# Icelk/fractal-renderer

Measured on AMD Instinct MI355X. Metric: pixel_iterations_per_sec, higher is better.
Workload: dtype f64

## Files before the change

### fractal-renderer_amd/csrc/fr_api.hip

```cpp
#include <hip/hip_runtime.h>

#include <atomic>
#include <cmath>
#include <cstddef>
#include <cstdint>
#include <cstdio>
#include <cstdlib>
#include <cstring>
#include <mutex>
#include <shared_mutex>
#include <string>
#include <vector>

#include "fr_ctx.h"

static_assert(sizeof(fr_config) == 104 && offsetof(fr_config, limit) == 16 && offsetof(fr_config, inside) == 72 &&
                  offsetof(fr_config, primary_color) == 74 && offsetof(fr_config, color_weight) == 80 &&
                  offsetof(fr_config, julia_set) == 88,
              "fr_config must stay the #[repr(C)] image of calc::Config");
static_assert(sizeof(fr_render_opts) == 32, "fr_render_opts is part of the ABI");

namespace fr {

namespace {
// ... 358 lines not shown
            slot_cv.notify_all();
        }
        s->busy = true;
        pending = s->pending;
        s->pending = false;
    }
    if (pending) e = hipEventSynchronize(s->done);
    if (e != hipSuccess) {
        {
            std::lock_guard<std::mutex> lk(palette_mu);
            s->busy = false;
        }
        slot_cv.notify_all();
        return fail_hip(e, "survivor-list buffer");
    }
    *out = s;
    return FR_OK;
}

void Ctx::release_surv(SurvSlot *slot, hipStream_t st) {
    if (!slot) return;
    const bool recorded = slot->done && hipEventRecord(slot->done, st) == hipSuccess;
    if (!recorded) (void)hipStreamSynchronize(st);
    {
        std::lock_guard<std::mutex> lk(palette_mu);
        slot->pending = recorded;
        slot->busy = false;
    }
    slot_cv.notify_all();
}

namespace {

int init_primary_locked(int device) {
    int n = 0;
    hipError_t e = hipGetDeviceCount(&n);
    if (e != hipSuccess || n <= 0) {
        (void)hipGetLastError();
        return fail(FR_ERR_NO_DEVICE, "no HIP device available (libfractal_hip has no CPU fallback)");
    }
    if (device < 0) device = g_primary_inited ? g_primary.hip_device : 0;
    if (device >= n) return fail(FR_ERR_NO_DEVICE, "device index out of range");
    if (g_primary_inited && g_primary.hip_device == device) return FR_OK;
    if (g_primary_inited) {
        g_primary.destroy();
        g_primary_inited = false;
    }
    static std::once_flag once;
    std::call_once(once, [] { atexit([] { g_process_exiting.store(true); }); });
    int rc = g_primary.create(device);
    if (rc != FR_OK) {
        g_primary.destroy();
        return rc;
    }
    g_primary_inited = true;
    return FR_OK;
}

}

int primary(Ctx **out) {
    {
        std::lock_guard<std::mutex> lk(g_primary_mu);
        if (!g_primary_inited) {
            int rc = init_primary_locked(-1);
            if (rc != FR_OK) return rc;
        }
    }
    HIP_TRY(hipSetDevice(g_primary.hip_device));
    *out = &g_primary;
    return FR_OK;
}

Ctx *primary_if_created() {
    std::lock_guard<std::mutex> lk(g_primary_mu);
    return g_primary_inited ? &g_primary : nullptr;
}

void fill_params(const fr_config *cfg, const Opts &o, fr_kparams &p) {
    memset(&p, 0, sizeof p);
    p.algo = cfg->algo;
    p.width = cfg->width;
    p.height = cfg->height;
    p.iterations = cfg->iterations;
    p.limit = cfg->limit;
    p.stable_limit = cfg->stable_limit;
    p.pos_re = cfg->pos.re;
    p.pos_im = cfg->pos.im;
    p.scale_re = cfg->scale.re;
    p.scale_im = cfg->scale.im;
    p.exposure = cfg->exposure;
    p.julia_re = cfg->julia_set.re;
    p.julia_im = cfg->julia_set.im;
    p.inside = cfg->inside ? 1u : 0u;
    p.smooth = cfg->smooth ? 1u : 0u;
    p.prim[0] = cfg->primary_color.r;
    p.prim[1] = cfg->primary_color.g;
    p.prim[2] = cfg->primary_color.b;
    p.sec[0] = cfg->secondary_color.r;
    p.sec[1] = cfg->secondary_color.g;
    p.sec[2] = cfg->secondary_color.b;
    for (int k = 0; k < 3; k++) {
        p.prim_f[k] = (double)p.prim[k];
        p.sec_f[k] = (double)p.sec[k];
    }
    p.iterations_f64 = (double)cfg->iterations;
    const uint32_t n = cfg->iterations;
    p.inv_iterations = (n != 0 && (n & (n - 1)) == 0) ? 1.0 / (double)n : 0.0;
    p.ncols = cfg->width;
    p.nrows = 0;
    p.x_first = 0;
    p.x_stride = 1;
    p.block_rows = 1;
    p.y_first = 0;
    p.y_stride = 1;
    p.refill_minrun = o.refill_minrun < 0 ? 32u : (uint32_t)o.refill_minrun;
    p.refill_quit16 = o.refill_quit16 < 0 ? 8u : (uint32_t)o.refill_quit16;
    p.queue_minrun = (o.refill_minrun < 0 || (o.tile >= 11 && o.tile <= 16)) ? 8u : (uint32_t)o.refill_minrun;
    p.first_keep = ((o.tile >= 11 && o.tile <= 16) && o.refill_quit16 > 0) ? 4u * (uint32_t)o.refill_quit16 : 0u;
    p.two_pass_cap = ((o.tile >= 11 && o.tile <= 16) && o.refill_minrun > 0) ? (uint32_t)o.refill_minrun : 0u;
    p.queue_want = (o.refill_quit16 < 0 || (o.tile >= 11 && o.tile <= 16)) ? 24u : (64u * (uint32_t)o.refill_quit16 + 15u) / 16u;
    {
        static const int dbg_want = getenv("FR_DEBUG_QUEUE_WANT") ? atoi(getenv("FR_DEBUG_QUEUE_WANT")) : 0;
        static const int dbg_minrun = getenv("FR_DEBUG_QUEUE_MINRUN") ? atoi(getenv("FR_DEBUG_QUEUE_MINRUN")) : -1;
        if (dbg_want > 0 && dbg_want <= 64) p.queue_want = (uint32_t)dbg_want;
        if (dbg_minrun >= 0) p.queue_minrun = (uint32_t)dbg_minrun;
    }
    {
        static const int dbg_ablate = getenv("FR_DEBUG_ABLATE") ? atoi(getenv("FR_DEBUG_ABLATE")) : 0;
        p.debug_ablate = (uint32_t)dbg_ablate & 3u;
    }
    p.cycle_shortcut = (o.cycle_shortcut && cfg->iterations < (1u << 30)) ? 1u : 0u;
    p.filt_k = n != 0 ? cfg->exposure / (double)n : 0.0;
    const bool filter_ok = o.colour_filter && cfg->smooth && n != 0 && std::isfinite(cfg->exposure) &&
                           std::fabs(p.filt_k) <= 1e100 && cfg->stable_limit >= 0.0;
    p.colour_filter = filter_ok ? 1u : 0u;
    const double ak = std::fabs(p.filt_k);
    p.colour_filter32 = (filter_ok && o.colour_filter == 1 && n < (1u << 24) && ak >= 0x1p-60 && ak <= 0x1p60) ? 1u : 0u;
    p.filt_k32 = (float)p.filt_k;
    p.filt_c32 = p.colour_filter32 ? std::nextafterf((float)(ak * FR_NU_BRACKET * (1.0 + 0x1p-9)), INFINITY) : 0.0f;
    for (int k = 0; k < 3; k++) {
        p.filt_d[k] = p.prim_f[k] * ak * FR_NU_BRACKET * (1.0 + 0x1p-20);
        p.filt_d32[k] = p.colour_filter32 ? std::nextafterf((float)(p.prim_f[k] * ak * FR_NU_BRACKET * (1.0 + 0x1p-10)), INFINITY) : 0.0f;
        p.prim32[k] = (float)p.prim[k];
    }
    const double lo = std::fmax(cfg->stable_limit, 2.0) * (1.0 + 0x1p-20);
    p.filt_lo32 = (p.colour_filter32 && lo < 1e30) ? std::nextafterf((float)lo, INFINITY) : INFINITY;
}

void rows_params(const fr_config *cfg, const Opts &o, uint32_t y0, uint32_t y1, unsigned channels, fr_kparams &p) {
    fill_params(cfg, o, p);
    p.nrows = y1 - y0;
    p.y_first = y0;
    p.block_rows = p.nrows;
    p.y_stride = 0;
    p.out_rgba = channels == 4 ? 1u : 0u;
}

static double host_coord(double coord, double max, double offset, double pos, double scale) {
    return ((coord / max) - offset) / scale + pos;
}

constexpr uint32_t kSpecQuiet = 16;
constexpr uint32_t kSpecBlock = 16, kSpecMaxLen = 128;

static uint32_t spec_maxlen() {
// ... 1220 lines not shown
```

### fractal-renderer_amd/csrc/fr_kernels.h

```cpp
#ifndef FR_KERNELS_H
#define FR_KERNELS_H

#include <hip/hip_runtime.h>
#include <stdint.h>

struct fr_kparams {
    uint32_t algo;
    uint32_t width, height;
    uint32_t iterations;
    double limit, stable_limit;
    double pos_re, pos_im, scale_re, scale_im;
    double exposure;
    double julia_re, julia_im;
    uint32_t inside, smooth;
    uint32_t prim[3], sec[3];
    double prim_f[3], sec_f[3];
    double iterations_f64, inv_iterations;
    uint32_t ncols, nrows;
    uint32_t x_first, x_stride;
    uint32_t block_rows, y_first, y_stride;
    uint32_t out_in_place;
    uint32_t out_rgba;
    uint32_t loop_mode;
    double skip_t;
    uint32_t loop_spec;
    uint32_t loop_spec_max;
    uint32_t first_no_spec;
    const uint32_t *palette;
    uint32_t palette_entries;
    uint32_t refill_minrun, refill_quit16;
    uint32_t queue_minrun, queue_want;
    uint32_t cycle_shortcut;
    uint32_t colour_filter;
    uint32_t *work_counter;
    double filt_k;
    double filt_d[3];
    uint32_t colour_filter32;
    float filt_k32;
    float filt_c32;
    float filt_d32[3];
    float prim32[3];
    float filt_lo32;
    uint32_t first_cap;
    uint32_t first_keep;
    uint32_t two_pass_cap;
    uint32_t first_only;
    uint32_t second_v1;
    uint32_t first_one_band;
    uint32_t strip_tiles;
    uint32_t debug_ablate;
    uint32_t surv_sub_capacity;
    void *surv_z;
    uint32_t *surv_pos;
    uint32_t *surv_cnt;
    void *surv_c;
    uint32_t *surv_counts;
};

constexpr uint32_t FR_SURV_QUEUES = 64;
constexpr uint32_t FR_SURV_COUNT_STRIDE = 32;
constexpr uint32_t FR_SURV_CHUNK = 64;

constexpr double FR_NU_BRACKET = 0x1p-18;

enum fr_out_mode {
    FR_OUT_RGB = 0,
    FR_OUT_ESCAPE = 1,
    FR_OUT_COUNT = 2
};

constexpr uint32_t FR_COUNT_SLOTS = 512;

constexpr int kDeepWaves = 4;
constexpr int kDeepTileW = 8, kDeepTileH = 8;
constexpr int kDeepWavesX = 2, kDeepWavesY = 2;
constexpr int kDeepBlockW = kDeepTileW * kDeepWavesX, kDeepBlockH = kDeepTileH * kDeepWavesY;

struct fr_kout {
    uint8_t *rgb;
    double *z;
    uint32_t *iters;
    unsigned long long *count;
    unsigned long long *trace;
};

inline hipError_t fr_deep_grid(const fr_kparams &p, dim3 &grid, dim3 &block) {
    const uint64_t tiles = (((uint64_t)p.ncols + kDeepBlockW - 1) / kDeepBlockW) * (((uint64_t)p.nrows + kDeepBlockH - 1) / kDeepBlockH);
    if (tiles > 0x7FFFFFFFull) return hipErrorInvalidValue;
    grid = dim3((uint32_t)tiles);
    block = dim3(64 * kDeepWaves);
    return hipSuccess;
}

hipError_t fr_launch_escape(const fr_kparams &p, int precision, int mode, const fr_kout &out, int tile,
                            hipStream_t stream, const char **kernel_name);

hipError_t fr_launch_escape_dd(const fr_kparams &p, double pos_lo_re, double pos_lo_im, int mode, const fr_kout &out,
                               bool with_lo, hipStream_t stream, const char **kernel_name);

bool fr_wants_work_queue(const fr_kparams &p, int tile);

bool fr_wants_two_pass(fr_kparams &p, int precision, int tile, int hint = -1);
struct fr_two_pass_layout {
    size_t z_off, pos_off, cnt_off, c_off, counts_off, total;
};
fr_two_pass_layout fr_two_pass_bytes(const fr_kparams &p, int precision, uint32_t sub_capacity);

hipError_t fr_launch_view_sample(const fr_kparams &p, int precision, uint32_t side, uint32_t cap_s, uint32_t episode, uint32_t keep,
                                 unsigned long long *counters, unsigned long long *result, unsigned long long tag,
                                 hipStream_t stream);

hipError_t fr_launch_copy_out(const void *src, void *dst, size_t bytes, unsigned int *counter, unsigned long long *flag,
                              unsigned long long seq, hipStream_t stream);

constexpr uint32_t FR_MAX_PALETTE_ENTRIES = 1280;

hipError_t fr_launch_palette(const fr_kparams &p, uint32_t *palette, hipStream_t stream);

hipError_t fr_launch_colour(const fr_kparams &p, const double *z, const uint32_t *iters, size_t n, uint8_t *rgb,
                            hipStream_t stream);

hipError_t fr_launch_escape_extend(const fr_kparams &p, int precision, uint32_t from_iterations, double *z, uint32_t *iters,
                                   hipStream_t stream, const char **kernel_name);
hipError_t fr_launch_escape_extend_dd(const fr_kparams &p, double pos_lo_re, double pos_lo_im, uint32_t from_iterations,
                                      double *z, uint32_t *iters, hipStream_t stream, const char **kernel_name);

hipError_t fr_launch_colour_rows(const fr_kparams &p, const double *z, uint32_t z_width, const uint32_t *iters, size_t n,
                                 uint32_t channels, void *out, hipStream_t stream);

hipError_t fr_launch_box_filter(const void *src, uint32_t width, uint64_t rows, uint32_t s, uint32_t bpp, void *dst,
                                hipStream_t stream);

hipError_t fr_launch_colour_filter(const fr_kparams &p, const double *z, uint32_t z_width, const uint32_t *iters, uint32_t width,
                                   uint64_t rows, uint32_t s, uint32_t bpp, void *dst, hipStream_t stream);

hipError_t fr_launch_view_stats(const double *z, uint32_t z_width, const uint32_t *iters, size_t n, double stable_limit,
                                uint32_t iterations, void *stats, hipStream_t stream);

hipError_t fr_launch_recursive_batch(uint32_t iterations, const double *start, const double *c, size_t n,
// ... 11 lines not shown
```

### fractal-renderer_amd/csrc/fr_kernels.hip

```cpp
#include "fr_kernels.h"

#include <cmath>

#include <cstdlib>

#include "fr_launch.h"
#include "fr_math.h"

namespace {

#include "fr_colour.h"

constexpr int kWaves = 4;



#define FR_ORBIT_IT_R(SFX, S, D)                           \
    "v_add_" SFX " %[t], %[r2" S "], -%[i2" S "]\n"        \
    "v_add_" SFX " %[x], %[re" S "], %[re" S "]\n"         \
    "v_add_" SFX " %[re" D "], %[t], %[cre]\n"             \
    "v_mul_" SFX " %[x], %[x], %[im" S "]\n"               \
    "v_add_" SFX " %[im" D "], %[x], %[cim]\n"             \
    "v_mul_" SFX " %[r2" D "], %[re" D "], %[re" D "]\n"   \
    "v_mul_" SFX " %[i2" D "], %[im" D "], %[im" D "]\n"
// ... 319 lines not shown
    "v_cmp_lt_" SFX " vcc, %[t4lim], %[t]\n"                                       \
    "s_cbranch_vccnz .Lslow_%=\n"                                                  \
    SP_ARM                                                                         \
    "s_branch .Lfast_%=\n"                                                         \
    FR_ORBIT_RECORD("R", "0") SLOW_RECORDS CYC_H SP_BODY                           \
    ".Ldone_%=:\n"                                                                 \
    "s_mov_b64 exec, %[sorig]\n"

#define FR_SC_CYC_CHECK(EQ, TAG)                   \
    EQ " %[scyc], %[X], %[Xs]\n"                   \
    EQ " vcc, %[Y], %[Ys]\n"                       \
    "s_and_b64 %[scyc], %[scyc], vcc\n"            \
    "s_cbranch_scc1 .Lcyc" TAG "_%=\n"             \
    ".Lcyccont" TAG "_%=:\n"                       \
    "s_cmp_ge_u32 %[si], %[snext]\n"               \
    "s_cbranch_scc1 .Lsave" TAG "_%=\n"            \
    ".Lsavecont" TAG "_%=:\n"

#define FR_SC_CYC_SAVE(MOV, TAG)                   \
    ".Lsave" TAG "_%=:\n"                          \
    MOV " %[Xs], %[X]\n"                           \
    MOV " %[Ys], %[Y]\n"                           \
    "v_mov_b32 %[vsaved], %[si]\n"                 \
    "s_lshl_b32 %[snext], %[snext], 1\n"           \
    "s_branch .Lsavecont" TAG "_%=\n"

#define FR_SC_CYC_HANDLER(TAG)                     \
    ".Lcyc" TAG "_%=:\n"                           \
    "s_or_b32 %[stmp], %[si], 0x80000000\n"        \
    "s_mov_b64 %[sprev], exec\n"                   \
    "s_mov_b64 exec, %[scyc]\n"                    \
    "v_mov_b32 %[it], %[stmp]\n"                   \
    "s_andn2_b64 exec, %[sprev], %[scyc]\n"        \
    "s_cbranch_execz .Ldone_%=\n"                  \
    "s_bcnt1_i32_b64 %[scnt], exec\n"              \
    "s_cmp_gt_u32 %[scnt], %[thr]\n"               \
    "s_cbranch_scc1 .Lcyccont" TAG "_%=\n"         \
    "s_cmp_lt_u32 %[si], %[minrun]\n"              \
    "s_cbranch_scc1 .Lcyccont" TAG "_%=\n"         \
    "s_branch .Ldone_%=\n"

#define FR_SC_ASM_M4_(SFX, CYC_F, CYC_S, CYC_H, SP_INIT, SP_ARM, SP_ENTRY, SP_BODY)                 \
    FR_SC_ASM(SFX, "4", FR_SC_ITS4(SFX),                    \
              FR_SC_CHECKED_STEP(SFX, "A") FR_SC_CHECKED_STEP(SFX, "B") FR_SC_CHECKED_STEP(SFX, "C") \
                  FR_SC_CHECKED_STEP(SFX, "D"),                                                     \
              FR_ORBIT_RECORD("A", "0") FR_ORBIT_RECORD("B", "1") FR_ORBIT_RECORD("C", "2")         \
                  FR_ORBIT_RECORD("D", "3"),                                                        \
              CYC_F, CYC_S, CYC_H, SP_INIT, SP_ARM, SP_ENTRY, SP_BODY)
#define FR_SC_ASM_M2_(SFX, CYC_F, CYC_S, CYC_H)                                            \
    FR_SC_ASM(SFX, "2", FR_SC_ITS2(SFX),                                        \
              FR_SC_CHECKED_STEP(SFX, "A") FR_SC_CHECKED_STEP(SFX, "B"),                    \
              FR_ORBIT_RECORD("A", "0") FR_ORBIT_RECORD("B", "1"), CYC_F, CYC_S, CYC_H, "", "", FR_SC_NOSPEC_ENTRY, "")
#define FR_SC_ASM_M4(SFX) FR_SC_ASM_M4_(SFX, "", "", "", "", "", FR_SC_NOSPEC_ENTRY, "")
#define FR_SC_ASM_M2(SFX) FR_SC_ASM_M2_(SFX, "", "", "")
#define FR_SC_ASM_M4_SPEC(SFX, MOV)                                                                 \
    FR_SC_ASM_M4_(SFX, "", "", "", "s_min_u32 %[sspec], %[specq], %[n]\n" "s_max_u32 %[lcap], %[lcap], " FR_SPEC_MSTR "\n", FR_SC_SPEC_ARM, FR_SC_SPEC_ENTRY(FR_SPEC_MSTR), \
                  FR_SC_SPEC_BODY(SFX, MOV, FR_SPEC_MSTR, FR_SC_SPEC_REST))
#define FR_SC_CYC_HANDLERS(MOV) \
    FR_SC_CYC_HANDLER("F") FR_SC_CYC_HANDLER("S") FR_SC_CYC_SAVE(MOV, "F") FR_SC_CYC_SAVE(MOV, "S")
#define FR_SC_ASM_M4_CYC(SFX, EQ, MOV) \
    FR_SC_ASM_M4_(SFX, FR_SC_CYC_CHECK(EQ, "F"), FR_SC_CYC_CHECK(EQ, "S"), FR_SC_CYC_HANDLERS(MOV), "", "", FR_SC_NOSPEC_ENTRY, "")
#define FR_SC_ASM_M2_CYC(SFX, EQ, MOV) \
    FR_SC_ASM_M2_(SFX, FR_SC_CYC_CHECK(EQ, "F"), FR_SC_CYC_CHECK(EQ, "S"), FR_SC_CYC_HANDLERS(MOV))

template <typename T>
struct ScalableRange;
template <>
struct ScalableRange<double> {
    static constexpr double lo = 0x1p-300, hi = 0x1p400;
};
template <>
struct ScalableRange<float> {
    static constexpr float lo = 0x1p-30f, hi = 0x1p30f;
};

template <typename T>
__device__ __forceinline__ bool lane_is_scalable(T re0, T im0, T cre, T cim) {
    constexpr T lo = ScalableRange<T>::lo, hi = ScalableRange<T>::hi;
    auto c_ok = [=](T v) { return __builtin_fabs(v) >= lo && __builtin_fabs(v) <= hi; };
    auto s_ok = [=](T v) { return v == (T)0 || c_ok(v); };
    return c_ok(cre) && c_ok(cim) && s_ok(re0) && s_ok(im0);
}

template <typename T, int M, bool CYC>
__device__ __forceinline__ uint32_t orbit_scaled_run(uint32_t iterations, T &X, T &Y, T &A, T &B, T c2re, T c2im,
                                                     T squared, T skip_t, EpisodeCtl ctl, uint32_t &completed,
                                                     T *pXs = nullptr, T *pYs = nullptr,
                                                     uint32_t *saved_index = nullptr, uint32_t spec_quiet = 0u,
                                                     uint32_t spec_maxlen = 0u) {
    uint32_t it;
    T t, q;
    T X1, Y1, A1, B1;
    uint32_t sspec;
    uint32_t specq = __builtin_amdgcn_readfirstlane(spec_quiet ? spec_quiet : 0xFFFFFFFFu);
    uint32_t lcap = __builtin_amdgcn_readfirstlane(spec_maxlen);
    T Xs = CYC ? *pXs : T(0), Ys = CYC ? *pYs : T(0);
    uint32_t vsaved = 0xFFFFFFFFu;
    uint32_t snext = 32u;
    unsigned long long sorig, sprev, sdiff, scyc;
    uint32_t si, stmp, nrem, scnt;
    const uint32_t n = __builtin_amdgcn_readfirstlane(iterations);
    const uint32_t thr = __builtin_amdgcn_readfirstlane(ctl.thr), minrun = __builtin_amdgcn_readfirstlane(ctl.minrun);
    const T lim4_v = (T)4 * squared, t4_v = (T)4 * skip_t;
#define FR_SC_OUTPUTS                                                                                           \
    [X] "+v"(X), [Y] "+v"(Y), [A] "+v"(A), [B] "+v"(B), [it] "=&v"(it), [t] "=&v"(t), [q] "=&v"(q),             \
        [sorig] "=&s"(sorig), [sprev] "=&s"(sprev), [sdiff] "=&s"(sdiff), [si] "=&s"(si), [stmp] "=&s"(stmp),   \
        [nrem] "=&s"(nrem), [scnt] "=&s"(scnt)
#define FR_SC_INPUTS                                                                                            \
    [c2re] "v"(c2re), [c2im] "v"(c2im), [lim4] "s"(lim4), [t4lim] "s"(t4lim), [n] "s"(n), [thr] "s"(thr),       \
        [minrun] "s"(minrun)
#define FR_SC_OPERANDS : FR_SC_OUTPUTS : FR_SC_INPUTS : "vcc", "scc"
#define FR_SC_OPERANDS_SPEC                                                                                     \
    : FR_SC_OUTPUTS, [X1] "=&v"(X1), [Y1] "=&v"(Y1), [A1] "=&v"(A1), [B1] "=&v"(B1), [sspec] "=&s"(sspec),      \
      [specq] "+&s"(specq), [lcap] "+&s"(lcap)                                                                  \
    : FR_SC_INPUTS                                                                                              \
    : "vcc", "scc"
#define FR_SC_OPERANDS_CYC                                                                                      \
    : FR_SC_OUTPUTS, [scyc] "=&s"(scyc), [Xs] "+v"(Xs), [Ys] "+v"(Ys), [vsaved] "+v"(vsaved), [snext] "+s"(snext) \
    : FR_SC_INPUTS                                                                                              \
    : "vcc", "scc"
    const auto lim4 = uniform_bits<T>(lim4_v), t4lim = uniform_bits<T>(t4_v);
    if constexpr (sizeof(T) == 8) {
        if constexpr (M == 4 && CYC)
            asm volatile(FR_SC_ASM_M4_CYC("f64", "v_cmp_eq_u64", "v_mov_b64") FR_SC_OPERANDS_CYC);
        else if constexpr (M == 4)
            asm volatile(FR_SC_ASM_M4_SPEC("f64", "v_mov_b64") FR_SC_OPERANDS_SPEC);
        else if constexpr (CYC)
            asm volatile(FR_SC_ASM_M2_CYC("f64", "v_cmp_eq_u64", "v_mov_b64") FR_SC_OPERANDS_CYC);
        else
            asm volatile(FR_SC_ASM_M2("f64") FR_SC_OPERANDS);
    } else {
        if constexpr (M == 4 && CYC)
            asm volatile(FR_SC_ASM_M4_CYC("f32", "v_cmp_eq_u32", "v_mov_b32") FR_SC_OPERANDS_CYC);
        else if constexpr (M == 4)
            asm volatile(FR_SC_ASM_M4_SPEC("f32", "v_mov_b32") FR_SC_OPERANDS_SPEC);
        else if constexpr (CYC)
            asm volatile(FR_SC_ASM_M2_CYC("f32", "v_cmp_eq_u32", "v_mov_b32") FR_SC_OPERANDS_CYC);
        else
            asm volatile(FR_SC_ASM_M2("f32") FR_SC_OPERANDS);
    }
    (void)scyc;
    (void)snext;
    (void)X1, (void)Y1, (void)A1, (void)B1, (void)sspec, (void)specq, (void)lcap;
    if constexpr (CYC) {
        *pXs = Xs;
        *pYs = Ys;
        *saved_index = vsaved;
    }
    completed = si;
    return it;
}

template <typename T, int M>
__device__ __forceinline__ uint32_t orbit_scaled(uint32_t iterations, T &re, T &im, T cre, T cim, T squared,
                                                 T skip_t, T &r2, T &i2, uint32_t spec_quiet = 0u, uint32_t spec_maxlen = 0u) {
    T X = re + re, Y = im + im, A = X * X, B = Y * Y;
    uint32_t completed;
    const uint32_t it = orbit_scaled_run<T, M, false>(iterations, X, Y, A, B, cre + cre, cim + cim, squared, skip_t,
                                               EpisodeCtl{0, 0}, completed, nullptr, nullptr, nullptr, spec_quiet, spec_maxlen);
    re = X * (T)0.5;
    im = Y * (T)0.5;
    r2 = re * re;
    i2 = im * im;
    return it;
}

template <typename T>
__device__ __forceinline__ uint32_t orbit_auto(uint32_t loop_mode, uint32_t iterations, T &re, T &im, T cre, T cim,
                                               T squared, T skip_t, T &r2, T &i2, int strip_scalable = -1,
                                               uint32_t spec_quiet = 0u, uint32_t spec_maxlen = 0u) {
    if (loop_mode != 0 && strip_scalable != 0) {
        bool all_ok = strip_scalable == 1;
        if (strip_scalable < 0) all_ok = __ballot(!lane_is_scalable<T>(re, im, cre, cim)) == 0ull;
        if (all_ok) {
            if (loop_mode == 4) return orbit_scaled<T, 4>(iterations, re, im, cre, cim, squared, skip_t, r2, i2, spec_quiet, spec_maxlen);
            return orbit_scaled<T, 2>(iterations, re, im, cre, cim, squared, skip_t, r2, i2);
        }
    }
    return orbit<T>(iterations, re, im, cre, cim, squared, r2, i2, spec_quiet);
}

__device__ __forceinline__ double coord_to_space(double coord, double max, double offset, double pos,
                                                 double scale) {
    return ((coord / max) - offset) / scale + pos;
}

__device__ __forceinline__ void store_pixel(uint32_t ncols, uint32_t out_rgba, uint8_t *base, uint32_t row, uint32_t col,
                                            const uint8_t rgb[3]) {
    const uint64_t k = (uint64_t)row * ncols + col;
    if (out_rgba) {
        reinterpret_cast<uint32_t *>(base)[k] =
            (uint32_t)rgb[0] | ((uint32_t)rgb[1] << 8) | ((uint32_t)rgb[2] << 16) | 0xFF000000u;
    } else {
        uint8_t *o = base + 3ull * k;
        o[0] = rgb[0];
        o[1] = rgb[1];
        o[2] = rgb[2];
    }
}
__device__ __forceinline__ void store_pixel(const fr_kparams &p, uint8_t *base, uint32_t row, uint32_t col, const uint8_t rgb[3]) {
    store_pixel(p.ncols, p.out_rgba, base, row, col, rgb);
}

typedef const __attribute__((address_space(4))) fr_kparams *KArgs;
#define FR_COLD_PARAMS(NAME)                                                          \
    KArgs NAME = (KArgs)__builtin_amdgcn_kernarg_segment_ptr();  \
    asm volatile("" : "+s"(NAME))

__device__ __forceinline__ unsigned long long ballot64(bool b) { return __builtin_amdgcn_ballot_w64(b); }

__device__ __forceinline__ bool lane_in(unsigned long long m) { return __builtin_amdgcn_inverse_ballot_w64(m); }

struct Filter32 {
    float lo, k, c, p0, p1, p2;
};
__device__ __forceinline__ uint32_t cvt_pk_u8_at(float v, uint32_t acc, int K) {
    return __builtin_amdgcn_cvt_pk_u8_f32(v, (uint32_t)K, acc);
}
__device__ __forceinline__ bool colour_fast32(const Filter32 &f, float d32, float itp1, uint32_t &lo) {
    const float l1 = __builtin_amdgcn_logf(d32);
    const float nu32 = __builtin_amdgcn_logf(l1 * 0.25f);
    const float m = (itp1 - nu32) * f.k;
    const float w = __builtin_fmaf(__builtin_fabsf(m), 0x1p-20f, f.c);
    const float ml = m - w, mh = m + w;
    lo = cvt_pk_u8_at(__builtin_fmaf(f.p2, ml, -0.5f), cvt_pk_u8_at(__builtin_fmaf(f.p1, ml, -0.5f), cvt_pk_u8_at(__builtin_fmaf(f.p0, ml, -0.5f), 0u, 0), 1), 2);
    const uint32_t hi = cvt_pk_u8_at(__builtin_fmaf(f.p2, mh, -0.5f), cvt_pk_u8_at(__builtin_fmaf(f.p1, mh, -0.5f), cvt_pk_u8_at(__builtin_fmaf(f.p0, mh, -0.5f), 0u, 0), 1), 2);
    return lo == hi;
}

__device__ __forceinline__ void store_packed(uint8_t *base, uint32_t off, uint32_t packed, uint32_t bpp) {
    if (bpp == 4u) {
        const uint32_t v = packed | 0xFF000000u;
        asm volatile("s_nop 4\n\tglobal_store_dword %0, %1, %2" : : "v"(off), "v"(v), "s"(base) : "memory");
    } else {
        asm volatile("s_nop 4\n\tglobal_store_short %0, %1, %2\n\tglobal_store_byte_d16_hi %0, %1, %2 offset:2" : : "v"(off), "v"(packed), "s"(base) : "memory");
    }
}

struct TileOut {
    uint8_t *base;
    uint32_t lane_off, bpp;
    bool narrow, fast_colour;
};

template <typename T>
__device__ __forceinline__ uint32_t colour_packed(bool valid, bool fast_colour, T re, T im, T r2, T i2, uint32_t iters,
                                                  const double *lds_tab, const uint32_t *palette) {
    uint32_t packed = 0;
    unsigned long long todo = ballot64(valid);
    if (fast_colour) {
        Filter32 f;
        {
            FR_COLD_PARAMS(kp);
            f.lo = kp->filt_lo32, f.k = kp->filt_k32, f.c = kp->filt_c32;
            f.p0 = kp->prim32[0], f.p1 = kp->prim32[2], f.p2 = kp->prim32[1];
        }
        float d32;
        if constexpr (sizeof(T) == 8)
            d32 = (float)(r2 + i2);
        else
            d32 = r2 + i2;
        const unsigned long long outside = ballot64(valid && d32 >= f.lo);
        if (outside != 0ull) {
            uint32_t pk;
            const bool decided = colour_fast32(f, d32, (float)(iters + 1u), pk);
            const bool ok = lane_in(outside) && d32 <= 0x1.ffffep119f && decided;
            packed = ok ? pk : 0u;
            todo &= ~ballot64(ok);
        }
    }
    if (todo != 0ull) {
        bool inside_done = false;
        if (lane_in(todo)) {
            double dist;
            if constexpr (sizeof(T) == 8) {
                dist = (double)(r2 + i2);
            } else {
                const double zre = (double)re, zim = (double)im;
                dist = zre * zre + zim * zim;
            }
            FR_COLD_PARAMS(kp);
            inside_done = !(dist > kp->stable_limit);
            if (inside_done && kp->inside)
                packed = sat_u8_dev(kp->sec_f[0] * dist) | (sat_u8_dev(kp->sec_f[2] * dist) << 8) | (sat_u8_dev(kp->sec_f[1] * dist) << 16);
        }
        todo &= ~ballot64(inside_done);
    }
    if (todo != 0ull) {
        if (lane_in(todo)) {
            FR_COLD_PARAMS(kp);
            const ColourConsts cc = make_colour_consts(*kp);
            uint8_t rgb[3];
            colour_pixel<T>(cc, re, im, r2, i2, iters, lds_tab, palette, rgb);
            packed = (uint32_t)rgb[0] | ((uint32_t)rgb[1] << 8) | ((uint32_t)rgb[2] << 16);
        }
    }
    return packed;
}

template <typename T, int MODE>
__device__ __forceinline__ void render_pixel(const fr_kparams &p, const fr_kout &out, const double *s_tab,
                                             const uint32_t *s_pal, double sre, double sim, bool valid,
                                             uint32_t cx, uint32_t r, uint32_t lane, uint32_t r_out,
                                             int strip_scalable = -1, const TileOut *to = nullptr) {
    double zre = 0.0, zim = 0.0;
    T tre = 0, tim = 0, tr2 = 0, ti2 = 0;
    uint32_t iters = 0;
    const bool escape_algo = p.algo == 0  || p.algo == 2 ;
    if (valid && escape_algo) {
        const double cre = p.algo == 0 ? sre : p.julia_re;
        const double cim = p.algo == 0 ? sim : p.julia_im;
        if constexpr (sizeof(T) == 8) {
            tre = sre;
            tim = sim;
            iters = orbit_auto<double>(p.loop_mode, p.iterations, tre, tim, cre, cim, p.limit * p.limit, p.skip_t,
                                       tr2, ti2, strip_scalable, p.loop_spec, p.loop_spec_max);
            zre = tre;
            zim = tim;
        } else {
            tre = (float)sre, tim = (float)sim;
            const float lim = (float)p.limit;
            iters = orbit_auto<float>(p.loop_mode, p.iterations, tre, tim, (float)cre, (float)cim, lim * lim,
                                      (float)p.skip_t, tr2, ti2, strip_scalable, p.loop_spec, p.loop_spec_max);
            zre = (double)tre;
            zim = (double)tim;
        }
    }

    if constexpr (MODE == FR_OUT_RGB) {
        if (to != nullptr) {
            uint32_t packed = 0;
            if (escape_algo) packed = colour_packed<T>(valid, to->fast_colour, tre, tim, tr2, ti2, iters, s_tab, s_pal);
            if (valid) {
                if (to->narrow) {
                    store_packed(to->base, to->lane_off, packed, to->bpp);
                } else {
                    const uint8_t rgb[3] = {(uint8_t)packed, (uint8_t)(packed >> 8), (uint8_t)(packed >> 16)};
                    store_pixel(p, out.rgb, r_out, cx, rgb);
                }
            }
        } else if (valid) {
            uint8_t rgb[3] = {0, 0, 0};
            if (escape_algo) {
                const ColourConsts cc = make_colour_consts(p);
                colour_pixel<T>(cc, tre, tim, tr2, ti2, iters, s_tab, s_pal, rgb);
            }
            store_pixel(p, out.rgb, r_out, cx, rgb);
        }
    } else if constexpr (MODE == FR_OUT_ESCAPE) {
        if (valid) {
            const uint64_t k = (uint64_t)r * p.ncols + cx;
            if (out.z) {
                out.z[2 * k] = zre;
                out.z[2 * k + 1] = zim;
            }
            if (out.iters) out.iters[k] = iters;
        }
    } else {
        unsigned long long n = 0;
        if (valid && escape_algo) n = iters < p.iterations ? (unsigned long long)iters + 1ull : p.iterations;
        for (int off = 32; off > 0; off >>= 1) n += __shfl_down(n, off, 64);
        if (lane == 0 && n) atomicAdd(out.count + ((blockIdx.x + 131u * blockIdx.y) % FR_COUNT_SLOTS), n);
    }
}

template <typename T, int TW, int TH, int WX, int WY, int MODE>
__global__ __launch_bounds__(64 * kWaves) void escape_kernel(const fr_kparams p, const fr_kout out) {
    static_assert(TW * TH == 64 && WX * WY == kWaves, "one lane per pixel, 4 waves per workgroup");
    constexpr int BW = TW * WX, BH = TH * WY;
    __shared__ double s_tab[FR_LOG2_N * 3];
    __shared__ double s_re[BW];
    __shared__ double s_im[BH];

    const uint32_t tid = threadIdx.x;
    const uint32_t tiles_x = (p.ncols + BW - 1) / BW;
    const uint32_t bx = blockIdx.x % tiles_x, by = blockIdx.x / tiles_x;
    const uint32_t col0 = bx * BW, row0 = by * BH;

    if (MODE == FR_OUT_RGB) {
        const double *gt = &g_log2_tab[0][0];
        for (uint32_t k = tid; k < FR_LOG2_N * 3; k += 64 * kWaves) s_tab[k] = gt[k];
    }
    if (tid < BW + BH) {
        const double width = (double)p.width, height = (double)p.height;
        if (tid < BW) {
            const uint32_t x = p.x_first + (col0 + tid) * p.x_stride;
            s_re[tid] = coord_to_space((double)x, height, (width / height) / 2.0, p.pos_re, p.scale_re);
        } else {
            const uint32_t r = row0 + (tid - BW);
            const uint32_t y = p.y_first + (r / p.block_rows) * p.y_stride + r % p.block_rows;
            s_im[tid - BW] = coord_to_space((double)y, height, 0.5, p.pos_im, p.scale_im);
        }
    }
    __syncthreads();

    const uint32_t wave = tid >> 6, lane = tid & 63;
    const uint32_t lx = (wave % WX) * TW + lane % TW;
    const uint32_t ly = (wave / WX) * TH + lane / TW;
    const uint32_t cx = col0 + lx, r = row0 + ly;
    const bool valid = cx < p.ncols && r < p.nrows;
    render_pixel<T, MODE>(p, out, s_tab, nullptr, s_re[lx], s_im[ly], valid, cx, r, lane, r);
}

template <typename T>
__device__ __forceinline__ bool coords_admissible(bool julia, double julia_re, double julia_im, double coord, bool relevant) {
    constexpr T lo = ScalableRange<T>::lo, hi = ScalableRange<T>::hi;
    const T v = (T)coord;
    const T av = __builtin_fabs(v);
    const bool in_range = av >= lo && av <= hi;
    bool lane_ok;
    if (julia) {
        const T jr = __builtin_fabs((T)julia_re), ji = __builtin_fabs((T)julia_im);
        lane_ok = (v == (T)0 || in_range) && jr >= lo && jr <= hi && ji >= lo && ji <= hi;
    } else {
        lane_ok = in_range;
    }
    return __ballot(relevant && !lane_ok) == 0ull;
}
template <typename T>
__device__ __forceinline__ bool coords_admissible(const fr_kparams &p, double coord, bool relevant) {
    return coords_admissible<T>(p.algo == 2, p.julia_re, p.julia_im, coord, relevant);
}

template <typename T>
__device__ __forceinline__ bool strip_is_scalable(const fr_kparams &p, double coord_lane, uint32_t tile0, uint32_t row0,
                                                  uint32_t lane) {
    const bool relevant = lane >= 56 ? (row0 + (lane - 56) < p.nrows) : (tile0 * 8u + lane < p.ncols);
    return coords_admissible<T>(p, coord_lane, relevant);
}


template <typename T, int MODE, int kStripTiles>
__global__ __launch_bounds__(64) void escape_strip_kernel(const fr_kparams p, const fr_kout out) {
    __shared__ double s_tab[(FR_LOG2_N * 3 * 8 > FR_MAX_PALETTE_ENTRIES * 4 ? FR_LOG2_N * 3 * 8 : FR_MAX_PALETTE_ENTRIES * 4) / 8];
    const uint32_t tid = threadIdx.x;
    const uint32_t *s_pal = nullptr;
    if (MODE == FR_OUT_RGB) {
        if (p.palette != nullptr) {
            uint32_t *dst = reinterpret_cast<uint32_t *>(s_tab);
            for (uint32_t k = tid; k < p.palette_entries; k += 64) dst[k] = p.palette[k];
            s_pal = dst;
        } else if (p.smooth) {
            const double *gt = &g_log2_tab[0][0];
            for (uint32_t k = tid; k < FR_LOG2_N * 3; k += 64) s_tab[k] = gt[k];
        }
        __syncthreads();
    }
    const uint32_t lane = tid;
    const uint32_t row0 = (blockIdx.y + gridDim.y * blockIdx.z) * 8u;
    if (row0 >= p.nrows) return;
    const uint32_t lx = lane & 7u, ly = lane >> 3;
    const uint32_t r = row0 + ly;
    const double width = (double)p.width, height = (double)p.height;

    static_assert(kStripTiles <= 7, "lanes 56-63 are the row lanes");
    const bool row_lane = lane >= 56;
    const uint32_t tile0 = blockIdx.x * kStripTiles;
    uint32_t coord_u;
    if (row_lane) {
        const uint32_t rr = row0 + (lane - 56);
        coord_u = p.y_first + (rr / p.block_rows) * p.y_stride + rr % p.block_rows;
    } else {
        coord_u = p.x_first + (tile0 * 8u + lane) * p.x_stride;
    }
    const double coord_lane = coord_to_space((double)coord_u, height, row_lane ? 0.5 : (width / height) / 2.0,
                                             row_lane ? p.pos_im : p.pos_re, row_lane ? p.scale_im : p.scale_re);
    const double sim = __shfl(coord_lane, 56 + ly, 64);
    uint32_t out_row0 = row0;
    if (p.out_in_place) out_row0 = p.y_first + (row0 / p.block_rows) * p.y_stride + row0 % p.block_rows;
    const uint32_t r_out = out_row0 + ly;
    const int strip_scalable = (p.loop_mode != 0 && strip_is_scalable<T>(p, coord_lane, tile0, row0, lane)) ? 1 : 0;
    TileOut to;
    to.bpp = p.out_rgba ? 4u : 3u;
    to.narrow = (uint64_t)p.ncols * to.bpp * 8u <= 0xFFFFFFFFull;
    to.lane_off = ly * (p.ncols * to.bpp) + lx * to.bpp;
    to.fast_colour = p.colour_filter32 && p.smooth && p.palette == nullptr;
    uint8_t *const strip_base = MODE == FR_OUT_RGB ? out.rgb + ((uint64_t)out_row0 * p.ncols + (uint64_t)tile0 * 8u) * to.bpp : nullptr;

    for (int k = 0; k < kStripTiles; k++) {
        const uint32_t col0 = (tile0 + k) * 8u;
        if (col0 >= p.ncols) break;
        const double sre = __shfl(coord_lane, k * 8 + lx, 64);
        const uint32_t cx = col0 + lx;
        const bool valid = cx < p.ncols && r < p.nrows;
        to.base = strip_base + (size_t)((uint32_t)k * 8u * to.bpp);
        render_pixel<T, MODE>(p, out, s_tab, s_pal, sre, sim, valid, cx, r, lane, r_out, strip_scalable, MODE == FR_OUT_RGB ? &to : nullptr);
    }
}

__device__ __forceinline__ uint32_t wave_max_u32(uint32_t v) {
    for (int off = 32; off > 0; off >>= 1) {
        const uint32_t o = __shfl_xor(v, off, 64);
        v = o > v ? o : v;
    }
    return v;
}

template <typename T>
struct Pair;
template <>
struct Pair<float> {
    typedef float2 type;
};
template <>
struct Pair<double> {
    typedef double2 type;
};

template <typename T>
__device__ __forceinline__ bool coord_is_scalable(bool julia, double coord) {
    constexpr T lo = ScalableRange<T>::lo, hi = ScalableRange<T>::hi;
    const T v = (T)coord;
    const T av = __builtin_fabs(v);
    const bool in_range = av >= lo && av <= hi;
    return julia ? (v == (T)0 || in_range) : in_range;
}

template <typename T, int M, int kStripTiles, int kBands>
__global__ __launch_bounds__(64) void escape_first_v1_kernel(const fr_kparams p, const fr_kout out) {
    __shared__ uint32_t s_palette[FR_MAX_PALETTE_ENTRIES];
    const double *const s_tab = &g_log2_tab[0][0];
    typedef typename Pair<T>::type T2;
    static_assert(kStripTiles <= 8 && kBands <= 8, "one column / one row coordinate per lane");
    const uint32_t lane = threadIdx.x;
    const uint32_t lx = lane & 7u, ly = lane >> 3;
    const uint32_t *s_pal = nullptr;
    uint32_t row0, tile0, ncols, nrows, bpp, lane_pitch;
    double cols, rows;
    bool cols_scalable;
    unsigned long long bad_rows;
    bool narrow;
    {
        FR_COLD_PARAMS(kp);
        const auto &P = *kp;
        if (P.palette != nullptr) {
            const uint32_t n = P.palette_entries;
            const uint32_t *src = P.palette;
            for (uint32_t k = lane; k < n; k += 64) s_palette[k] = src[k];
            s_pal = s_palette;
            __syncthreads();
        }
        row0 = (blockIdx.y + gridDim.y * blockIdx.z) * (8u * kBands);
        nrows = P.nrows, ncols = P.ncols;
        if (row0 >= nrows) return;
        const double width = (double)P.width, height = (double)P.height;
        tile0 = blockIdx.x * kStripTiles;
        const uint32_t block_rows = P.block_rows;
        const uint32_t x = P.x_first + (tile0 * 8u + lane) * P.x_stride;
        cols = coord_to_space((double)x, height, (width / height) / 2.0, P.pos_re, P.scale_re);
        const uint32_t rr = row0 + lane;
        const uint32_t y = P.y_first + (rr / block_rows) * P.y_stride + rr % block_rows;
        rows = coord_to_space((double)y, height, 0.5, P.pos_im, P.scale_im);
        bpp = P.out_rgba ? 4u : 3u;
        narrow = (uint64_t)ncols * bpp * 8u <= 0xFFFFFFFFull;
        lane_pitch = ly * (ncols * bpp) + lx * bpp;
        const bool is_julia = P.algo == 2;
        bool c_ok = true;
        if (is_julia) {
            constexpr T lo = ScalableRange<T>::lo, hi = ScalableRange<T>::hi;
            const T jr = __builtin_fabs((T)P.julia_re), ji = __builtin_fabs((T)P.julia_im);
            c_ok = jr >= lo && jr <= hi && ji >= lo && ji <= hi;
        }
        const bool col_relevant = lane < 8u * kStripTiles && tile0 * 8u + lane < ncols;
        const bool row_relevant = lane < 8u * kBands && rr < nrows;
        cols_scalable = c_ok && __ballot(col_relevant && !coord_is_scalable<T>(is_julia, cols)) == 0ull;
        bad_rows = __ballot(row_relevant && !coord_is_scalable<T>(is_julia, rows));
    }
    const uint32_t k1 = p.first_cap, cap = p.iterations, keep = p.first_keep;
    const bool julia = p.algo == 2;
// ... 2228 lines not shown
```

Baseline: 5475 billion.

## Hoist per-strip constants and lazily stage log2 table in strip kernel

Computes per-strip loop constants (squared limit, scaled limits, julia and c_im values, the x offset) once per block instead of once per pixel, and passes them into a new strip-specialised orbit path. It stages the smooth-colour log2 table into LDS only when some lane actually needs the slow colour path, skipping the upfront copy and barrier. It also simplifies row-coordinate computation when all 8 rows fall in one block. The point is to cut per-pixel setup and prologue work, at the cost of extra register pressure and a barrier inside divergent-looking but wave-uniform code.

```diff
diff --git a/fractal-renderer_amd/csrc/fr_api.hip b/fractal-renderer_amd/csrc/fr_api.hip
--- a/fractal-renderer_amd/csrc/fr_api.hip
+++ b/fractal-renderer_amd/csrc/fr_api.hip
@@ -464,6 +464,7 @@
     p.algo = cfg->algo;
     p.width = cfg->width;
     p.height = cfg->height;
+    p.x_offset = ((double)cfg->width / (double)cfg->height) / 2.0;
     p.iterations = cfg->iterations;
     p.limit = cfg->limit;
     p.stable_limit = cfg->stable_limit;
diff --git a/fractal-renderer_amd/csrc/fr_kernels.h b/fractal-renderer_amd/csrc/fr_kernels.h
--- a/fractal-renderer_amd/csrc/fr_kernels.h
+++ b/fractal-renderer_amd/csrc/fr_kernels.h
@@ -55,6 +55,7 @@
     uint32_t *surv_cnt;
     void *surv_c;
     uint32_t *surv_counts;
+    double x_offset;
 };
 
 constexpr uint32_t FR_SURV_QUEUES = 64;
diff --git a/fractal-renderer_amd/csrc/fr_kernels.hip b/fractal-renderer_amd/csrc/fr_kernels.hip
--- a/fractal-renderer_amd/csrc/fr_kernels.hip
+++ b/fractal-renderer_amd/csrc/fr_kernels.hip
@@ -425,12 +425,21 @@
     return c_ok(cre) && c_ok(cim) && s_ok(re0) && s_ok(im0);
 }
 
+template <typename T>
+struct ScaledLimits {
+    typename UBits<T>::type lim4, t4lim;
+};
+template <typename T>
+__device__ __forceinline__ ScaledLimits<T> scaled_limits(T squared, T skip_t) {
+    return ScaledLimits<T>{uniform_bits<T>((T)4 * squared), uniform_bits<T>((T)4 * skip_t)};
+}
+
 template <typename T, int M, bool CYC>
 __device__ __forceinline__ uint32_t orbit_scaled_run(uint32_t iterations, T &X, T &Y, T &A, T &B, T c2re, T c2im,
                                                      T squared, T skip_t, EpisodeCtl ctl, uint32_t &completed,
                                                      T *pXs = nullptr, T *pYs = nullptr,
                                                      uint32_t *saved_index = nullptr, uint32_t spec_quiet = 0u,
-                                                     uint32_t spec_maxlen = 0u) {
+                                                     uint32_t spec_maxlen = 0u, const ScaledLimits<T> *pre = nullptr) {
     uint32_t it;
     T t, q;
     T X1, Y1, A1, B1;
@@ -444,7 +453,6 @@
     uint32_t si, stmp, nrem, scnt;
     const uint32_t n = __builtin_amdgcn_readfirstlane(iterations);
     const uint32_t thr = __builtin_amdgcn_readfirstlane(ctl.thr), minrun = __builtin_amdgcn_readfirstlane(ctl.minrun);
-    const T lim4_v = (T)4 * squared, t4_v = (T)4 * skip_t;
 #define FR_SC_OUTPUTS                                                                                           \
     [X] "+v"(X), [Y] "+v"(Y), [A] "+v"(A), [B] "+v"(B), [it] "=&v"(it), [t] "=&v"(t), [q] "=&v"(q),             \
         [sorig] "=&s"(sorig), [sprev] "=&s"(sprev), [sdiff] "=&s"(sdiff), [si] "=&s"(si), [stmp] "=&s"(stmp),   \
@@ -462,7 +470,8 @@
     : FR_SC_OUTPUTS, [scyc] "=&s"(scyc), [Xs] "+v"(Xs), [Ys] "+v"(Ys), [vsaved] "+v"(vsaved), [snext] "+s"(snext) \
     : FR_SC_INPUTS                                                                                              \
     : "vcc", "scc"
-    const auto lim4 = uniform_bits<T>(lim4_v), t4lim = uniform_bits<T>(t4_v);
+    const ScaledLimits<T> lims = pre != nullptr ? *pre : scaled_limits<T>(squared, skip_t);
+    const auto lim4 = lims.lim4, t4lim = lims.t4lim;
     if constexpr (sizeof(T) == 8) {
         if constexpr (M == 4 && CYC)
             asm volatile(FR_SC_ASM_M4_CYC("f64", "v_cmp_eq_u64", "v_mov_b64") FR_SC_OPERANDS_CYC);
@@ -586,9 +595,18 @@
     bool narrow, fast_colour;
 };
 
+struct LazyTable {
+    double *lds;
+    bool staged;
+};
+__device__ __forceinline__ void stage_log2_table(double *lds) {
+    const double *gt = &g_log2_tab[0][0];
+    for (uint32_t k = threadIdx.x; k < FR_LOG2_N * 3; k += 64) lds[k] = gt[k];
+    __syncthreads();
+}
 template <typename T>
 __device__ __forceinline__ uint32_t colour_packed(bool valid, bool fast_colour, T re, T im, T r2, T i2, uint32_t iters,
-                                                  const double *lds_tab, const uint32_t *palette) {
+                                                  const double *lds_tab, const uint32_t *palette, LazyTable *lazy_tab = nullptr) {
     uint32_t packed = 0;
     unsigned long long todo = ballot64(valid);
     if (fast_colour) {
@@ -630,6 +648,10 @@
         todo &= ~ballot64(inside_done);
     }
     if (todo != 0ull) {
+        if (lazy_tab != nullptr && !lazy_tab->staged) {
+            stage_log2_table(lazy_tab->lds);
+            lazy_tab->staged = true;
+        }
         if (lane_in(todo)) {
             FR_COLD_PARAMS(kp);
             const ColourConsts cc = make_colour_consts(*kp);
@@ -641,16 +663,95 @@
     return packed;
 }
 
+template <typename T>
+struct StripConsts {
+    T squared, skip_t;
+    ScaledLimits<T> lims;
+    T jre, j2re;
+    T cim, c2im;
+    LazyTable tab;
+};
+
+template <typename T>
+__device__ __forceinline__ T own_value(T v) {
+    asm("" : "+v"(v));
+    return v;
+}
+
+template <typename T>
+__device__ __forceinline__ void strip_c_im(StripConsts<T> &sc, bool julia, T jim, T im) {
+    if (julia) {
+        sc.cim = jim;
+        sc.c2im = jim + jim;
+    } else {
+        sc.cim = own_value<T>(im);
+        sc.c2im = own_value<T>(im + im);
+    }
+}
+
+template <typename T>
+__device__ __forceinline__ T unread_value() {
+    T v;
+    asm volatile("" : "=v"(v));
+    return v;
+}
+
+template <typename T>
+__device__ __forceinline__ uint32_t orbit_strip(const fr_kparams &p, const StripConsts<T> &sc, bool julia, bool scalable, T &re,
+                                                T &im, T &r2, T &i2) {
+    uint32_t completed;
+    if (p.loop_mode != 0 && scalable) {
+        T X = re + re, Y = im + im, A = X * X, B = Y * Y;
+        T c2re;
+        if (julia)
+            c2re = own_value<T>(sc.j2re);
+        else
+            c2re = own_value<T>(X);
+        uint32_t it;
+        if (p.loop_mode == 4)
+            it = orbit_scaled_run<T, 4, false>(p.iterations, X, Y, A, B, c2re, sc.c2im, sc.squared, sc.skip_t, EpisodeCtl{0, 0},
+                                               completed, nullptr, nullptr, nullptr, p.loop_spec, p.loop_spec_max, &sc.lims);
+        else
+            it = orbit_scaled_run<T, 2, false>(p.iterations, X, Y, A, B, c2re, sc.c2im, sc.squared, sc.skip_t, EpisodeCtl{0, 0},
+                                               completed, nullptr, nullptr, nullptr, 0u, 0u, &sc.lims);
+        re = X * (T)0.5;
+        im = Y * (T)0.5;
+        r2 = re * re;
+        i2 = im * im;
+        return it;
+    }
+    T cre;
+    if (julia)
+        cre = own_value<T>(sc.jre);
+    else
+        cre = own_value<T>(re);
+    r2 = re * re;
+    i2 = im * im;
+    return orbit_run<T>(p.iterations, re, im, cre, sc.cim, sc.squared, r2, i2, EpisodeCtl{0, 0}, completed, p.loop_spec);
+}
+
 template <typename T, int MODE>
 __device__ __forceinline__ void render_pixel(const fr_kparams &p, const fr_kout &out, const double *s_tab,
                                              const uint32_t *s_pal, double sre, double sim, bool valid,
                                              uint32_t cx, uint32_t r, uint32_t lane, uint32_t r_out,
-                                             int strip_scalable = -1, const TileOut *to = nullptr) {
+                                             int strip_scalable = -1, const TileOut *to = nullptr,
+                                             StripConsts<T> *sc = nullptr) {
     double zre = 0.0, zim = 0.0;
     T tre = 0, tim = 0, tr2 = 0, ti2 = 0;
     uint32_t iters = 0;
     const bool escape_algo = p.algo == 0  || p.algo == 2 ;
-    if (valid && escape_algo) {
+    if (sc != nullptr) {
+        if (escape_algo) {
+            tre = unread_value<T>(), tim = unread_value<T>(), tr2 = unread_value<T>(), ti2 = unread_value<T>();
+            iters = unread_value<uint32_t>();
+            if (valid) {
+                tre = (T)sre, tim = (T)sim;
+                iters = orbit_strip<T>(p, *sc, p.algo == 2, strip_scalable == 1, tre, tim, tr2, ti2);
+            }
+            zre = (double)tre;
+            zim = (double)tim;
+        }
+    } else if (valid && escape_algo) {
         const double cre = p.algo == 0 ? sre : p.julia_re;
         const double cim = p.algo == 0 ? sim : p.julia_im;
         if constexpr (sizeof(T) == 8) {
@@ -673,7 +774,8 @@
     if constexpr (MODE == FR_OUT_RGB) {
         if (to != nullptr) {
             uint32_t packed = 0;
-            if (escape_algo) packed = colour_packed<T>(valid, to->fast_colour, tre, tim, tr2, ti2, iters, s_tab, s_pal);
+            if (escape_algo)
+                packed = colour_packed<T>(valid, to->fast_colour, tre, tim, tr2, ti2, iters, s_tab, s_pal, sc ? &sc->tab : nullptr);
             if (valid) {
                 if (to->narrow) {
                     store_packed(to->base, to->lane_off, packed, to->bpp);
@@ -783,34 +885,44 @@
             uint32_t *dst = reinterpret_cast<uint32_t *>(s_tab);
             for (uint32_t k = tid; k < p.palette_entries; k += 64) dst[k] = p.palette[k];
             s_pal = dst;
-        } else if (p.smooth) {
-            const double *gt = &g_log2_tab[0][0];
-            for (uint32_t k = tid; k < FR_LOG2_N * 3; k += 64) s_tab[k] = gt[k];
-        }
-        __syncthreads();
-    }
+            __syncthreads();
+        }
+    }
+    StripConsts<T> sc;
+    sc.tab.lds = s_tab;
+    sc.tab.staged = !(MODE == FR_OUT_RGB && p.palette == nullptr && p.smooth);
     const uint32_t lane = tid;
     const uint32_t row0 = (blockIdx.y + gridDim.y * blockIdx.z) * 8u;
     if (row0 >= p.nrows) return;
     const uint32_t lx = lane & 7u, ly = lane >> 3;
     const uint32_t r = row0 + ly;
-    const double width = (double)p.width, height = (double)p.height;
+    const double height = (double)p.height;
+    const T lim = (T)p.limit;
+    sc.squared = lim * lim;
+    sc.skip_t = (T)p.skip_t;
+    sc.jre = (T)p.julia_re;
+    sc.j2re = sc.jre + sc.jre;
+    sc.lims = scaled_limits<T>(sc.squared, sc.skip_t);
 
     static_assert(kStripTiles <= 7, "lanes 56-63 are the row lanes");
     const bool row_lane = lane >= 56;
     const uint32_t tile0 = blockIdx.x * kStripTiles;
+    const uint32_t blk0 = row0 / p.block_rows, rem0 = row0 % p.block_rows;
+    const uint32_t y_row0 = p.y_first + blk0 * p.y_stride + rem0;
+    const bool one_block = p.block_rows - rem0 > 7u;
     uint32_t coord_u;
     if (row_lane) {
         const uint32_t rr = row0 + (lane - 56);
-        coord_u = p.y_first + (rr / p.block_rows) * p.y_stride + rr % p.block_rows;
+        coord_u = one_block ? y_row0 + (lane - 56) : p.y_first + (rr / p.block_rows) * p.y_stride + rr % p.block_rows;
     } else {
         coord_u = p.x_first + (tile0 * 8u + lane) * p.x_stride;
     }
-    const double coord_lane = coord_to_space((double)coord_u, height, row_lane ? 0.5 : (width / height) / 2.0,
+    const double coord_lane = coord_to_space((double)coord_u, height, row_lane ? 0.5 : p.x_offset,
                                              row_lane ? p.pos_im : p.pos_re, row_lane ? p.scale_im : p.scale_re);
     const double sim = __shfl(coord_lane, 56 + ly, 64);
+    strip_c_im<T>(sc, p.algo == 2, (T)p.julia_im, (T)sim);
     uint32_t out_row0 = row0;
-    if (p.out_in_place) out_row0 = p.y_first + (row0 / p.block_rows) * p.y_stride + row0 % p.block_rows;
+    if (p.out_in_place) out_row0 = y_row0;
     const uint32_t r_out = out_row0 + ly;
     const int strip_scalable = (p.loop_mode != 0 && strip_is_scalable<T>(p, coord_lane, tile0, row0, lane)) ? 1 : 0;
     TileOut to;
@@ -827,7 +939,7 @@
         const uint32_t cx = col0 + lx;
         const bool valid = cx < p.ncols && r < p.nrows;
         to.base = strip_base + (size_t)((uint32_t)k * 8u * to.bpp);
-        render_pixel<T, MODE>(p, out, s_tab, s_pal, sre, sim, valid, cx, r, lane, r_out, strip_scalable, MODE == FR_OUT_RGB ? &to : nullptr);
+        render_pixel<T, MODE>(p, out, s_tab, s_pal, sre, sim, valid, cx, r, lane, r_out, strip_scalable, MODE == FR_OUT_RGB ? &to : nullptr, &sc);
     }
 }
 
```

Measured after the change: 5483 billion, median of 2. No clear change (+0.1%).
